# franioli/icepy4d

Hardware: AMD Instinct MI355X
Metric: matched stereo image-pairs/sec (4096 kpts, 1080p) (higher is better)
Workload: dtype f32

## Files before the change

icepy4d_amd/_lib.py:

```python
from __future__ import annotations

import ctypes as C
import os
import subprocess
from typing import Optional

_HERE = os.path.dirname(os.path.abspath(__file__))
CSRC = os.path.join(_HERE, "csrc")
LIB_PATH = os.environ.get("ICEMATCH_LIB") or os.path.join(CSRC, "libicematch.so")

_lib: Optional[C.CDLL] = None


class IcematchError(RuntimeError):

    def __init__(self, what: str, rc: int, message: str):
        super().__init__(f"{what} failed ({rc}): {message}")
        self.what, self.rc = what, rc


class LightGlueConf(C.Structure):
    _fields_ = [("depth_confidence", C.c_double), ("width_confidence", C.c_double),
                ("filter_threshold", C.c_double), ("n_layers", C.c_int), ("pruning_min_kpts", C.c_int)]

# ... 6 lines not shown
_I = C.c_int
_F = C.c_float
_D = C.c_double
_L = C.c_longlong

SIGNATURES = {
    "im_version": [],
    "im_ctx_create": [_I, C.POINTER(_P)],
    "im_ctx_destroy": [_P],
    "im_last_error": [_P],
    "im_ctx_reserve": [_P, _I, _I, _I, _I],
    "im_profile_begin": [_P],
    "im_profile_end": [_P, C.c_char_p, C.c_size_t],
    "im_set_tensor": [_P, C.c_char_p, C.c_char_p, _P, C.c_size_t],
    "im_finalize_weights": [_P, C.c_char_p],
    "im_superpoint_forward": [_P, _P, _I, _I, _I, _I, _I, _F, _I, _I, _I, _P, _P, _P, _P, _P],
    "im_superpoint_candidates": [_P, _I, _P, _P],
    "im_lightglue_forward": [_P, _P, _P, _P, _P, C.POINTER(LightGlueConf), _P, _P, _P, _P, _P],
    "im_lightglue_forward_pairs": [_P, _I, _P, _P, _P, _P, C.POINTER(LightGlueConf), _P, _P, _P, _P, _P],
    "im_pack_records": [_P, _I, _P, _P, _P, _P, _I, _P, _P, _P],
    "im_superglue_forward": [_P, _P, _P, _P, _P, _P, C.POINTER(SuperGlueConf), _P, _P, _P, _P],
    "im_pack_record": [_P, _P, _P, _P, _P, _I, _P, _P],
    "im_debug_read": [_P, C.c_char_p, _P, C.c_size_t, _P],
    "im_debug_clock_probe": [_P, _I, _P, _P],
    "im_debug_guard_failures": [],
    "im_debug_guard_selftest": [_P, _P],
    "im_debug_guards_check": [_P, _P],
    "im_pyr_down": [_P, _P, _P, _I, _I, _I, _I, _P],
    "im_pyr_up": [_P, _P, _P, _I, _I, _I, _I, _P],
    "im_gemm_nt": [_P, _P, _P, _P, _P, _I, _I, _I, _F, _I, _P],
    "im_ffn_fused": [_P, _I, _P, _P, _P, _P, _P, _P, _P, _P, _I, _I, _P, _P],
    "im_conv3x3": [_P, _P, _P, _P, _P, _I, _I, _I, _I, _I, _I, _I, _P],
    "im_conv3x3_winograd": [_P, _P, _P, _P, _P, _I, _I, _I, _I, _I, _I, _I, _P],
    "im_flash_attn": [_P, _P, _P, _P, _P, _P, _I, _I, _I, _I, _F, _P],
    "im_nms": [_P, _P, _P, _I, _I, _I, _I, _P],
    "im_select_topk": [_P, _P, _I, _I, _I, _I, _F, _I, _P, _P, _P, _P],
    "im_sample_descriptors": [_P, _P, _I, _I, _I, _P, _P, _P, _P],
    "im_assign_from_sim": [_P, _P, _I, _I, _I, _P, _P, _F, _P, _P, _P, _P, _P],
    "im_log_optimal_transport": [_P, _P, _I, _I, _I, _F, _I, _P, _P],
    "im_merge_tile_matches": [_P, _I, _I, _P, _P, _P, _P, _P, _P, _P, _P, _P, _P, _P, _P],
    "im_gather_rows": [_P, _P, _I, _P, _I, _P, _P],
    "im_ransac_fundamental": [_P, _P, _P, _I, _I, C.c_double, C.c_uint, _P, _P, _P, _P],
    "im_ransac_essential": [_P, _P, _P, _I, _I, C.c_double, C.c_uint, _P, _P, _P, _P],
    "im_triangulate_linear": [_P, _P, _P, _P, _P, _I, _P, _P],
    "im_forient": [_P, _P, _I, _I, _I, _I, _P, _P],
    "im_template_match_oc": [_P, _P, _I, _I, _P, _I, _I, _I, _P, _P, _I, _I, _I, _I, _P, _P],
# ... 85 lines not shown
```

icepy4d_amd/csrc/block.h:

```cpp
#pragma once
#include "ctx.h"

namespace im {

struct BlockFfn {
    int act = 0;
    const float* w0 = nullptr; const float* w0p = nullptr;
    const float* b0 = nullptr;
    const float* ln_g = nullptr; const float* ln_b = nullptr;
    const float* w3 = nullptr; const float* w3p = nullptr;
    const float* b3 = nullptr;
    const char* name_fused = nullptr; const char* name_ffn0 = nullptr; const char* name_ffn3 = nullptr;
};

int launch_block_proj(im_ctx* ctx, hipStream_t s, const char* name, const GemmArgs& g, const float* wp_layers, int layer);

int launch_block_tail(im_ctx* ctx, hipStream_t s, const AttnArgs& at, const BlockFfn& f, const GemmArgs& base, float* x);

}
```

icepy4d_amd/csrc/block.hip:

```cpp
#include "block.h"

#include "lg_misc.h"
#include "workspace.h"

namespace im {

int launch_block_proj(im_ctx* ctx, hipStream_t s, const char* name, const GemmArgs& g, const float* wp_layers, int layer) {
    if (env_is_1("IM_PROJ_TILED")) {
        IM_LAUNCH(ctx, name, s, launch_gemm(g, s));
        return 0;
    }
    GemmArgs r = g;
    r.wp = reinterpret_cast<const unsigned char*>(wp_layers) + (size_t)layer * g.N * 256 * 6;
    IM_LAUNCH(ctx, name, s, launch_proj_rows(r, s));
    return 0;
}

int launch_block_tail(im_ctx* ctx, hipStream_t s, const AttnArgs& at, const BlockFfn& f, const GemmArgs& base, float* x) {
    Workspace* ws = ctx->ws;
    const long xb = (long)base.m_max * 256, hb = (long)base.m_max * 512;
    IM_LAUNCH(ctx, "attn_kv_planes", s, launch_attn_planes(at, s));
    IM_LAUNCH(ctx, at.cross ? "flash_attn_cross" : "flash_attn_self", s, launch_flash_attn(at, s));
    static const bool unfused = env_is_1("IM_FFN_UNFUSED");
    if (!unfused) {
        FfnArgs a;
        a.act = f.act; a.x = x; a.x_bstride = xb; a.att = at.out; a.att_bstride = xb;
        a.w0p = f.w0p; a.b0 = f.b0; a.ln_g = f.ln_g; a.ln_b = f.ln_b; a.w3p = f.w3p; a.b3 = f.b3;
        a.m_max = base.m_max; a.batch = base.batch; a.m_ptr = base.m_ptr; a.active = base.active; a.pstride = base.pstride;
        IM_LAUNCH(ctx, f.name_fused, s, launch_ffn_fused(a, s));
        return 0;
    }
    {
        GemmArgs g = base;
        g.A = x; g.a_bstride = xb; g.lda = 256; g.A1 = at.out; g.a1_bstride = xb; g.lda1 = 256; g.ksplit = 256;
        g.W = f.w0; g.ldw = 512; g.bias = f.b0; g.N = 512; g.K = 512;
        g.C = ws->h; g.c_bstride = hb; g.ldc = 512; g.epi = f.act == 1 ? EPI_BIAS_RELU : EPI_BIAS;
        IM_LAUNCH(ctx, f.name_ffn0, s, launch_gemm(g, s));
    }
    if (f.act == 0)
        IM_LAUNCH(ctx, "lg_layernorm_gelu", s, launch_layernorm_gelu(ws->h, hb, ws->st, base.batch, base.m_max, f.ln_g, f.ln_b, s));
    {
        GemmArgs g = base;
        g.A = ws->h; g.a_bstride = hb; g.lda = 512; g.W = f.w3; g.ldw = 512; g.bias = f.b3; g.N = 256; g.K = 512;
        g.C = x; g.c_bstride = xb; g.ldc = 256; g.R = x; g.r_bstride = xb; g.ldr = 256; g.epi = EPI_BIAS_RESID;
// ... 7 lines not shown
```

icepy4d_amd/csrc/capi.hip:

```cpp
#include "ctx.h"
#include "lg_misc.h"
#include "sp_post.h"
#include "workspace.h"

#include <algorithm>
#include <cstdio>
#include <cstdlib>
#include <cstring>

using namespace im;

template <int N, typename F>
static hipError_t with_uploads(const float* const (&src)[N], const size_t (&sizes)[N], hipStream_t st, F&& launch) {
    float* d[N] = {};
    hipError_t e = hipSuccess;
    for (int i = 0; i < N && e == hipSuccess; ++i) {
        e = hipMalloc(&d[i], sizes[i] * sizeof(float));
        if (e == hipSuccess) e = hipMemcpy(d[i], src[i], sizes[i] * sizeof(float), hipMemcpyHostToDevice);
    }
    if (e == hipSuccess) e = launch(d);
    const hipError_t e2 = hipStreamSynchronize(st);
    for (int i = 0; i < N; ++i) hipFree(d[i]);
    return e != hipSuccess ? e : e2;
}
// ... 150 lines not shown
        first = false;
    }
    out += "}";
    if (!buf || out.size() + 1 > cap) return ctx->fail(-60, "im_profile_end: buffer too small (%zu needed)", out.size() + 1);
    memcpy(buf, out.c_str(), out.size() + 1);
    return 0;
}

int im_debug_read(im_ctx* ctx, const char* name, float* d_dst, size_t nfloats, void* stream) {
    IM_CHECK_CTX(ctx);
    Workspace* ws = ctx->ws;
    if (!ws || !name) return ctx->fail(-51, "im_debug_read: no workspace");
    const size_t K = (size_t)ctx->max_kpts;
    const std::string nm = name;
    const float* src = nullptr;
    size_t avail = 0;
    if (nm == "lg_x") { src = ws->x[ctx->dbg_cur]; avail = 2 * K * 256; }
    else if (nm == "lg_cos") { src = ws->cs[ctx->dbg_cur]; avail = 2 * K * 32; }
    else if (nm == "lg_sin") { src = ws->sn[ctx->dbg_cur]; avail = 2 * K * 32; }
    else if (nm == "sim") { src = ws->sim; avail = K * K; }
    else if (nm == "md") { src = ws->md; avail = 2 * K * 256; }
    else if (nm == "sp_smap") { src = ws->smap; avail = ws->smap_floats; }
    else if (nm == "sp_nms") { src = ws->nms; avail = ws->smap_floats; }
    else return ctx->fail(-61, "im_debug_read: unknown buffer '%s'", name);
    if (nfloats > avail) return ctx->fail(-62, "im_debug_read: %zu floats requested, %zu available", nfloats, avail);
    IM_HIP(ctx, hipMemcpyAsync(d_dst, src, nfloats * sizeof(float), hipMemcpyDeviceToDevice, (hipStream_t)stream));
    IM_HIP(ctx, hipStreamSynchronize((hipStream_t)stream));
    return 0;
}

int im_debug_clock_probe(im_ctx* ctx, int arm, double* h_out, void* stream) {
    IM_CHECK_CTX(ctx);
    hipStream_t s = (hipStream_t)stream;
    const size_t bytes = (size_t)CLOCK_PROBE_SLOTS * 2 * sizeof(unsigned long long);
    if (arm == 1) {
        IM_GROW(ctx, ctx->grow(ctx->scratch.clock[0], bytes, "clock_probe_attention"), -22, "im_debug_clock_probe: allocation failed");
        IM_GROW(ctx, ctx->grow(ctx->scratch.clock[1], bytes, "clock_probe_convolution"), -22, "im_debug_clock_probe: allocation failed");
        IM_HIP(ctx, hipMemsetAsync(ctx->scratch.clock[0].p, 0, bytes, s));
        IM_HIP(ctx, hipMemsetAsync(ctx->scratch.clock[1].p, 0, bytes, s));
        IM_HIP(ctx, hipStreamSynchronize(s));
        ctx->clock_armed = true;
        return 0;
    }
    if (!ctx->scratch.clock[0].p || !h_out) return ctx->fail(-51, "im_debug_clock_probe: not armed");
    std::vector<unsigned long long> h((size_t)CLOCK_PROBE_SLOTS * 2);
    const void* src[2] = {ctx->scratch.clock[0].p, ctx->scratch.clock[1].p};
    for (int c = 0; c < 2; ++c) {
        IM_HIP(ctx, hipMemcpyAsync(h.data(), src[c], bytes, hipMemcpyDeviceToHost, s));
        IM_HIP(ctx, hipStreamSynchronize(s));
// ... 145 lines not shown
```

icepy4d_amd/csrc/gemm.hip:

```cpp
#include "bf16x3.h"
#include "common.h"
#include "kernels.h"

namespace im {

template <int BM, int BN, int BK, int EPI, bool BX>
__global__ __launch_bounds__(256) void gemm_nt_kernel(GemmArgs a) {
    constexpr int LDS_LD = BK + 4;
    constexpr int WM = BM / 2, WN = BN / 2;
    constexpr int MB = WM / 32, NB = WN / 32;
    constexpr int F4 = BK / 4;
    constexpr int A_IT = BM * F4 / 256, B_IT = BN * F4 / 256;
    constexpr int XS = BK * 2 + 16, XPA = BM * XS, XPB = BN * XS;
    __shared__ __attribute__((aligned(16))) float smem[BX ? 3 * (XPA + XPB) / 4 : (BM + BN) * LDS_LD];
    float* sA = smem;
    float* sB = smem + BM * LDS_LD;
    unsigned char* const xA = reinterpret_cast<unsigned char*>(smem);
    unsigned char* const xB = xA + 3 * XPA;

    const int gm = (a.m_max + BM - 1) / BM;
    const int z = blockIdx.y;
    const int pair = a.pair_batched ? z : (z >> 1);
    if (a.active && a.active[pair * a.pstride] == 0) return;
    const int M = a.m_ptr ? a.m_ptr[a.pair_batched ? z * a.pstride : (z >> 1) * a.pstride + (z & 1)] : a.m_max;
// ... 185 lines not shown
                if (rope) {
                    const __amdgpu_buffer_rsrc_t rCs = make_rsrc(a.cs + (long)z * a.enc_bstride, (unsigned)M * 128u);
                    const __amdgpu_buffer_rsrc_t rSn = make_rsrc(a.sn + (long)z * a.enc_bstride, (unsigned)M * 128u);
                    const unsigned ve = (rowl * 32 + (d >> 1)) * 4u;
#pragma unroll
                    for (int r = 0; r < 16; ++r) {
                        const unsigned so = ((r & 3) + 8 * (r >> 2)) * 128u;
                        const float cs = __uint_as_float(__builtin_amdgcn_raw_buffer_load_b32(rCs, ve, so, 0));
                        const float sn = __uint_as_float(__builtin_amdgcn_raw_buffer_load_b32(rSn, ve, so, 0));
                        const float val = acc[i][j][r] + bv;
                        const float partner = __shfl_xor(val, 1);
                        const float outv = (d & 1) ? (val * cs) + (partner * sn) : (val * cs) + ((-partner) * sn);
                        __builtin_amdgcn_raw_buffer_store_b32(__float_as_uint(outv), rD, vo, ((r & 3) + 8 * (r >> 2)) * 256u, 0);
                    }
                } else {
#pragma unroll
                    for (int r = 0; r < 16; ++r)
                        __builtin_amdgcn_raw_buffer_store_b32(__float_as_uint(scale * (acc[i][j][r] + bv)), rD, vo, ((r & 3) + 8 * (r >> 2)) * 256u, 0);
                }
            }
        }
}

namespace pr {
constexpr int BM = 32, NT = 512;
constexpr int PS = 528;
constexpr int PLANE = BM * PS;
constexpr int LDS_BYTES = 3 * PLANE;
constexpr unsigned TILE_BYTES = (256 / 16) * 3 * 1024;
}

#ifdef IM_PSTAMP
__device__ unsigned long long g_pstamp[4096 * 16];
#define P_STAMP(i) { if (wave == 0) { const unsigned long long ts_ = __builtin_amdgcn_s_memtime(); const int b_ = blockIdx.y * gridDim.x + blockIdx.x; if (lane == 0 && b_ < 4096) g_pstamp[b_ * 16 + (i)] = ts_; } }
extern "C" int im_debug_pstamps(unsigned long long* host, size_t n) {
    return (int)hipMemcpyFromSymbol(host, HIP_SYMBOL(g_pstamp), n * sizeof(unsigned long long));
}
#else
#define P_STAMP(i)
#endif

template <int EPI, int TILES>
__global__ __launch_bounds__(pr::NT, 4) void proj_rows_kernel(GemmArgs a) {
    using namespace pr;
    static_assert(EPI == EPI_QKV_ROPE || EPI == EPI_HEADS_QV, "the two projections of a LightGlue block");
    extern __shared__ __attribute__((aligned(16))) unsigned char psm[];
    const int z = blockIdx.y, pair = z >> 1;
    if (a.active && a.active[pair * a.pstride] == 0) return;
    const int M = a.m_ptr ? a.m_ptr[pair * a.pstride + (z & 1)] : a.m_max;
    const int m0 = blockIdx.x * BM;
    if (m0 >= M) return;
    const int tid = threadIdx.x, lane = tid & 63;
    const int wave = __builtin_amdgcn_readfirstlane(tid >> 6);
    const int c = lane & 31, hh = lane >> 5;
    const __amdgpu_buffer_rsrc_t rX = make_rsrc(a.A + (long)z * a.a_bstride, (unsigned)M * 1024u);
    const __amdgpu_buffer_rsrc_t rW = make_rsrc(a.wp, (unsigned)a.N * 256u * 6u);

    P_STAMP(0)
    u32x4 b0[3], b1[3], b2[3], b3[3];
#define PR_LOAD(b_, s_)                                                                                                          \
    {                                                                                                                            \
        const bool in_ = (s_) < TILES * 16;                                                                                      \
        const unsigned so_ = in_ ? (unsigned)((((s_) >> 4) * 8 + wave)) * TILE_BYTES + (unsigned)(((s_) & 15) * 3) * 1024u : 0u;   \
        const unsigned vo_ = in_ ? lane * 16u : 0x80000000u;     \
        _Pragma("unroll") for (int g = 0; g < 3; ++g) b_[g] = __builtin_amdgcn_raw_buffer_load_b128(rW, vo_, so_ + (unsigned)g * 1024u, 0); \
    }
    PR_LOAD(b0, 0)
    PR_LOAD(b1, 1)
    PR_LOAD(b2, 2)
    {
        float4 v[4];
#pragma unroll
        for (int i = 0; i < 4; ++i) {
            const int idx = tid + i * NT;
            v[i] = buf_load4(rX, (unsigned)((m0 + (idx >> 6)) * 256 + (idx & 63) * 4) * 4u, 0);
        }
#pragma unroll
        for (int i = 0; i < 4; ++i) {
            const int idx = tid + i * NT;
            unsigned h0, m0_, l0, h1, m1, l1;
            split2(v[i].x, v[i].y, h0, m0_, l0);
            split2(v[i].z, v[i].w, h1, m1, l1);
            unsigned char* d = psm + (idx >> 6) * PS + (idx & 63) * 8;
            *reinterpret_cast<u32x2*>(d) = u32x2{h0, h1};
            *reinterpret_cast<u32x2*>(d + PLANE) = u32x2{m0_, m1};
            *reinterpret_cast<u32x2*>(d + 2 * PLANE) = u32x2{l0, l1};
        }
    }
    __syncthreads();
    P_STAMP(1)

#define PR_SIX(b_, kc_)                                                                                              \
    {                                                                                                                \
        const unsigned char* ap = psm + c * PS + ((kc_) * 16 + hh * 8) * 2;                                          \
        const u32x4 ah = *reinterpret_cast<const u32x4*>(ap), am = *reinterpret_cast<const u32x4*>(ap + PLANE),   \
                     al = *reinterpret_cast<const u32x4*>(ap + 2 * PLANE);                                          \
        acc = mfma_bf(ah, b_[2], acc);                                                                              \
        acc = mfma_bf(al, b_[0], acc);                                                                              \
        acc = mfma_bf(am, b_[1], acc);                                                                              \
        acc = mfma_bf(ah, b_[1], acc);                                                                              \
        acc = mfma_bf(am, b_[0], acc);                                                                              \
        acc = mfma_bf(ah, b_[0], acc);                                                                              \
    }
#pragma unroll 1
    for (int j = 0; j < TILES; ++j) {
        const int tile = j * 8 + wave;
        f32x16 acc;
#pragma unroll
        for (int r = 0; r < 16; ++r) acc[r] = 0.f;
#pragma unroll 1
        for (int kc = 0; kc < 16; kc += 4) {
            const int s_ = j * 16 + kc;
            PR_LOAD(b3, s_ + 3)
            __builtin_amdgcn_sched_barrier(0);
            PR_SIX(b0, kc)
            __builtin_amdgcn_sched_barrier(0);
            PR_LOAD(b0, s_ + 4)
            __builtin_amdgcn_sched_barrier(0);
            PR_SIX(b1, kc + 1)
            __builtin_amdgcn_sched_barrier(0);
            PR_LOAD(b1, s_ + 5)
            __builtin_amdgcn_sched_barrier(0);
            PR_SIX(b2, kc + 2)
            __builtin_amdgcn_sched_barrier(0);
            PR_LOAD(b2, s_ + 6)
            __builtin_amdgcn_sched_barrier(0);
            PR_SIX(b3, kc + 3)
            __builtin_amdgcn_sched_barrier(0);
        }
        P_STAMP(2 + 2 * j)
        const int colbase = tile * 32;
        const int col = colbase + c;
        const float bv = a.bias ? a.bias[col] : 0.f;
        const unsigned rowl = m0 + 4 * hh;
        const int which = colbase >> 8, hd = colbase & 255;
        float* dst = a.q;
        if constexpr (EPI == EPI_QKV_ROPE) dst = which == 0 ? a.q : (which == 1 ? a.k : a.v);
        if constexpr (EPI == EPI_HEADS_QV) dst = which ? a.v : a.q;
        const __amdgpu_buffer_rsrc_t rD = make_rsrc(dst + (long)z * a.head_bstride + (long)(hd >> 6) * a.head_stride, (unsigned)M * 256u);
        const int d = (hd & 63) + c;
        const unsigned vo = (rowl * 64 + d) * 4u;
        float scale = a.alpha;
        if constexpr (EPI == EPI_QKV_ROPE) scale = 1.f;
        if constexpr (EPI == EPI_HEADS_QV) scale = which ? 1.f : a.alpha;
        const bool rope = EPI == EPI_QKV_ROPE && which < 2 && a.cs;
        if (rope) {
            const __amdgpu_buffer_rsrc_t rCs = make_rsrc(a.cs + (long)z * a.enc_bstride, (unsigned)M * 128u);
            const __amdgpu_buffer_rsrc_t rSn = make_rsrc(a.sn + (long)z * a.enc_bstride, (unsigned)M * 128u);
            const unsigned ve = (rowl * 32 + (d >> 1)) * 4u;
#pragma unroll
            for (int r = 0; r < 16; ++r) {
                const unsigned so = ((r & 3) + 8 * (r >> 2)) * 128u;
                const float cs = __uint_as_float(__builtin_amdgcn_raw_buffer_load_b32(rCs, ve, so, 0));
                const float sn = __uint_as_float(__builtin_amdgcn_raw_buffer_load_b32(rSn, ve, so, 0));
                const float val = acc[r] + bv;
                const float partner = __shfl_xor(val, 1);
                const float outv = (d & 1) ? (val * cs) + (partner * sn) : (val * cs) + ((-partner) * sn);
                __builtin_amdgcn_raw_buffer_store_b32(__float_as_uint(outv), rD, vo, ((r & 3) + 8 * (r >> 2)) * 256u, 0);
            }
        } else {
#pragma unroll
            for (int r = 0; r < 16; ++r)
                __builtin_amdgcn_raw_buffer_store_b32(__float_as_uint(scale * (acc[r] + bv)), rD, vo, ((r & 3) + 8 * (r >> 2)) * 256u, 0);
        }
        P_STAMP(3 + 2 * j)
    }
#undef PR_LOAD
#undef PR_SIX
}

template <int EPI, int TILES>
static hipError_t launch_proj_rows_t(const GemmArgs& a, hipStream_t s) {
    const dim3 grid((a.m_max + pr::BM - 1) / pr::BM, a.batch), block(pr::NT);
    return launch_dyn_lds<proj_rows_kernel<EPI, TILES>>(grid, block, pr::LDS_BYTES, s, a);
}

hipError_t launch_proj_rows(const GemmArgs& a, hipStream_t s) {
    if (!a.wp || a.K != 256 || a.lda != 256 || a.A1 || a.sel || a.w_bstride || a.n_ptr || a.pair_batched) return hipErrorInvalidValue;
    if (a.m_max <= 0 || a.batch <= 0) return hipSuccess;
    if (a.epi == EPI_QKV_ROPE && a.N == 768) return launch_proj_rows_t<EPI_QKV_ROPE, 3>(a, s);
    if (a.epi == EPI_HEADS_QV && a.N == 512) return launch_proj_rows_t<EPI_HEADS_QV, 2>(a, s);
    return hipErrorInvalidValue;
}

hipError_t launch_gemm(const GemmArgs& a, hipStream_t s) {
    if (a.K % 32 != 0 || (a.A1 && a.ksplit % 64 != 0)) return hipErrorInvalidValue;
    const int bm = a.big_tile ? 128 : 64, bn = bm;
    dim3 grid(((a.N + bn - 1) / bn) * ((a.m_max + bm - 1) / bm), a.batch), block(256);
    if (grid.x == 0) return hipSuccess;
#define IM_GEMM_CASE(E)                                                                  \
    case E:                                                                              \
// ... 23 lines not shown
```

icepy4d_amd/csrc/kernels.h:

```cpp
#pragma once
#include <hip/hip_runtime.h>
#include <stdint.h>
#include <cstdlib>
#include <vector>

#include "common.h"

namespace im {

inline bool env_is_1(const char* name) {
    const char* e = getenv(name);
    return e && e[0] == '1';
}
inline int env_int(const char* name) {
    const char* e = getenv(name);
    return e ? atoi(e) : 0;
}

inline hipError_t current_device(int* dev) {
    if (hipError_t e = hipGetDevice(dev); e != hipSuccess) return e;
    return (*dev < 0 || *dev >= IM_MAX_DEVICES) ? hipErrorInvalidDevice : hipSuccess;
}
inline hipError_t device_cu_count(int* n) {
    static int n_cu[IM_MAX_DEVICES] = {0};
// ... 34 lines not shown

struct GemmArgs {
    const float* A = nullptr;  long a_bstride = 0;  int lda = 0;
    const float* A1 = nullptr; long a1_bstride = 0; int lda1 = 0; int ksplit = 0;
    const float* W = nullptr;  int ldw = 0; long w_bstride = 0;
    const float* bias = nullptr;
    const int* sel = nullptr; long w_sel_stride = 0; long bias_sel_stride = 0;
    int N = 0, K = 0;
    int m_max = 0;
    const int* m_ptr = nullptr;
    const int* n_ptr = nullptr;
    const int* active = nullptr;
    int pstride = 2;
    int pair_batched = 0;
    int batch = 1;
    float alpha = 1.f;
    float* C = nullptr; long c_bstride = 0; int ldc = 0;
    const float* R = nullptr; long r_bstride = 0; int ldr = 0;
    float* q = nullptr; float* k = nullptr; float* v = nullptr; long head_bstride = 0; long head_stride = 0;
    const float* cs = nullptr; const float* sn = nullptr; long enc_bstride = 0;
    int epi = EPI_BIAS;
    int big_tile = 0;
    int bx = 0;
    const void* wp = nullptr;
};
hipError_t launch_gemm(const GemmArgs& a, hipStream_t s);
hipError_t launch_proj_rows(const GemmArgs& a, hipStream_t s);

struct FfnArgs {
    int act = 0;
    float* x = nullptr; long x_bstride = 0;
    const float* att = nullptr; long att_bstride = 0;
    const float* w0p = nullptr; const float* b0 = nullptr;
    const float* ln_g = nullptr; const float* ln_b = nullptr;
    const float* w3p = nullptr; const float* b3 = nullptr;
    int m_max = 0; int batch = 1;
    const int* m_ptr = nullptr;
    const int* active = nullptr;
    int pstride = 2;
};
hipError_t launch_ffn_fused(const FfnArgs& a, hipStream_t s);
std::vector<float> pack_frag_weights(const float* w, int n, int k);

struct AttnArgs {
    const float* q = nullptr; const float* k = nullptr; const float* v = nullptr;
    long bstride = 0; long hstride = 0;
    float* out = nullptr; long out_bstride = 0; int ldo = 256;
    const int* n_ptr = nullptr;
    int pstride = 2;
    int n_max = 0; int batch = 2; int heads = 4; int cross = 0;
    float scale = 1.f;
    const int* active = nullptr;
    float* part = nullptr;
    int* counters = nullptr;
    void* planes = nullptr;
    int f32_form = 0;
    unsigned long long* clock = nullptr;
};
static constexpr int CLOCK_PROBE_SLOTS = 4096;
static constexpr int ATTN_MAX_SPLIT = 4;
inline size_t attn_part_floats(int n_max, int batch, int heads) { return (size_t)ATTN_MAX_SPLIT * batch * heads * n_max * 66; }
inline size_t attn_planes_bytes(int n_max, int batch, int heads) { return (size_t)2 * batch * heads * n_max * 384; }
inline size_t attn_counter_ints(int n_max, int batch, int heads) { return (size_t)batch * heads * ((n_max + 127) / 128); }
bool attn_f32_form(const AttnArgs& a);
hipError_t launch_flash_attn(const AttnArgs& a, hipStream_t s);
hipError_t launch_attn_planes(const AttnArgs& a, hipStream_t s);
hipError_t launch_flash_attn_bx(const AttnArgs& a, hipStream_t s);

struct ConvArgs {
    const float* in = nullptr;
    const float* w = nullptr;
    const float* bias = nullptr;
    float* out = nullptr;
    int B = 1, H = 0, W = 0, Cin = 0, Cout = 0;
    int pool = 0;
    int relu = 1;
    const uint8_t* img = nullptr;
    int img_channels = 1;
// ... 16 lines not shown
```

icepy4d_amd/csrc/lightglue.hip:

```cpp
#include "block.h"
#include "lg_misc.h"
#include "workspace.h"

using namespace im;

static constexpr int ST_INTS = (int)(sizeof(LGState) / sizeof(int));

static int lg_block(im_ctx* ctx, hipStream_t s, int NI, int layer, bool cross, float* x, const float* cs, const float* sn) {
    Workspace* ws = ctx->ws;
    const LightGlueW& W = ctx->lg;
    const int K = ctx->max_kpts;
    const long xb = (long)K * 256;
    const int* n_ptr = ws->st->n;
    const int* active = &ws->st->active;
    GemmArgs base;
    base.m_max = K; base.m_ptr = n_ptr; base.active = active; base.pstride = ST_INTS; base.batch = NI; base.bx = 1;
    AttnArgs at;
    at.q = ws->q; at.k = cross ? ws->q : ws->k; at.v = ws->v; at.hstride = (long)K * 64; at.bstride = (long)K * 256;
    at.out = ws->att; at.out_bstride = xb; at.ldo = 256; at.n_ptr = n_ptr; at.pstride = ST_INTS; at.n_max = K; at.batch = NI; at.heads = 4;
    at.cross = cross ? 1 : 0; at.active = active; at.part = ws->attn_part; at.counters = ws->attn_cnt; at.planes = ws->attn_planes; at.clock = ctx->clock_of(0);
    GemmArgs g = base;
    g.A = x; g.a_bstride = xb; g.lda = 256; g.ldw = 256; g.K = 256;
    g.q = ws->q; g.v = ws->v; g.head_bstride = (long)K * 256; g.head_stride = (long)K * 64; g.big_tile = NI >= 4;
    if (!cross) {
        g.W = W.qkv_w + (long)layer * 768 * 256; g.bias = W.qkv_b + (long)layer * 768; g.N = 768; g.epi = EPI_QKV_ROPE;
        g.k = ws->k; g.cs = cs; g.sn = sn; g.enc_bstride = (long)K * 32;
        if (int rc = launch_block_proj(ctx, s, "lg_qkv_rope_gemm", g, W.qkv_wp, layer)) return rc;
        at.scale = 0.125f;
    } else {
        g.W = W.cqv_w + (long)layer * 512 * 256; g.bias = W.cqv_b + (long)layer * 512; g.N = 512; g.epi = EPI_HEADS_QV;
        g.alpha = (float)0.35355339059327373;
        if (int rc = launch_block_proj(ctx, s, "lg_proj_gemm", g, W.cqv_wp, layer)) return rc;
        at.scale = 1.f;
    }
    const LightGlueW::Ffn& F = cross ? W.cross_ffn : W.self_ffn;
    BlockFfn f;
    f.w0 = F.w0 + (long)layer * 512 * 512; f.w0p = F.w0p + (long)layer * 512 * 512 * 3 / 2; f.b0 = F.b0 + (long)layer * 512;
    f.ln_g = F.ln_g + (long)layer * 512; f.ln_b = F.ln_b + (long)layer * 512;
    f.w3 = F.w3 + (long)layer * 256 * 512; f.w3p = F.w3p + (long)layer * 256 * 512 * 3 / 2; f.b3 = F.b3 + (long)layer * 256;
    f.name_fused = "lg_ffn_fused"; f.name_ffn0 = "lg_ffn0_gemm"; f.name_ffn3 = "lg_ffn3_gemm";
    return launch_block_tail(ctx, s, at, f, base, x);
}

static int lightglue_forward(im_ctx* ctx, int n_pairs, const float* d_kpts, const float* d_desc, const int32_t* d_n, const float* h_size,
                             const im_lightglue_conf* conf, int32_t* d_matches, float* d_mscores, int32_t* d_prune, int32_t* d_info,
                             void* stream) {
    IM_CHECK_CTX(ctx);
    if (!ctx->lg.ready) return ctx->fail(-50, "im_lightglue_forward: weights not finalized");
    Workspace* ws = ctx->ws;
    if (!ws) return ctx->fail(-51, "im_lightglue_forward: call im_ctx_reserve first");
    if (n_pairs < 1 || n_pairs > ws->n_pairs || n_pairs > 64)
        return ctx->fail(-53, "im_lightglue_forward: %d pairs, the workspace was reserved for %d (max_images / 2)", n_pairs, ws->n_pairs);
    hipStream_t s = (hipStream_t)stream;
    const LightGlueW& W = ctx->lg;
    const int K = ctx->max_kpts;
// ... 98 lines not shown
```

include/icematch.h:

```cpp
#ifndef ICEMATCH_H
#define ICEMATCH_H

#include <stddef.h>
#include <stdint.h>

#ifdef __cplusplus
extern "C" {
#endif

typedef struct im_ctx im_ctx;

int im_version(void);
int im_ctx_create(int device, im_ctx** out);
void im_ctx_destroy(im_ctx* ctx);
const char* im_last_error(im_ctx* ctx);
int im_ctx_reserve(im_ctx* ctx, int max_h, int max_w, int max_images, int max_kpts);

int im_profile_begin(im_ctx* ctx);
int im_profile_end(im_ctx* ctx, char* buf, size_t cap);

int im_set_tensor(im_ctx* ctx, const char* model, const char* key, const float* h_data, size_t numel);
int im_finalize_weights(im_ctx* ctx, const char* model);

int im_superpoint_forward(im_ctx* ctx, const uint8_t* d_img, int n_images, int h, int w, int channels,
// ... 10 lines not shown
} im_lightglue_conf;
int im_lightglue_forward(im_ctx* ctx, const float* d_kpts, const float* d_desc, const int32_t* d_n,
                         const float* h_size, const im_lightglue_conf* conf,
                         int32_t* d_matches, float* d_mscores, int32_t* d_prune, int32_t* d_info, void* stream);

int im_lightglue_forward_pairs(im_ctx* ctx, int n_pairs, const float* d_kpts, const float* d_desc, const int32_t* d_n,
                               const float* h_size, const im_lightglue_conf* conf, int32_t* d_matches, float* d_mscores,
                               int32_t* d_prune, int32_t* d_info, void* stream);

typedef struct {
    int sinkhorn_iterations;
    double match_threshold;
    int n_layers;
} im_superglue_conf;
int im_superglue_forward(im_ctx* ctx, const float* d_kpts, const float* d_scores, const float* d_desc,
                         const int32_t* d_n, const float* h_shape, const im_superglue_conf* conf,
                         int32_t* d_matches, float* d_mscores, int32_t* d_info, void* stream);

int im_pack_record(im_ctx* ctx, const int32_t* d_n, const int32_t* d_matches0, const float* d_mscores0,
                   const int32_t* d_info, int epoch, int32_t* d_record, void* stream);
int im_pack_records(im_ctx* ctx, int n_pairs, const int32_t* d_n, const int32_t* d_matches, const float* d_mscores,
                    const int32_t* d_info, int first_epoch, int32_t* d_records, const float* d_kpts, void* stream);
int im_debug_read(im_ctx* ctx, const char* name, float* d_dst, size_t nfloats, void* stream);
int im_debug_clock_probe(im_ctx* ctx, int arm, double* h_out, void* stream);
int im_debug_guard_failures(void);
int im_debug_guard_selftest(im_ctx* ctx, void* stream);
int im_debug_guards_check(im_ctx* ctx, void* stream);

int im_gemm_nt(im_ctx* ctx, const float* d_a, const float* d_w, const float* d_bias, float* d_c,
               int m, int n, int k, float alpha, int big_tile, void* stream);
int im_ffn_fused(im_ctx* ctx, int act, float* d_x, const float* d_att, const float* h_w0, const float* h_b0, const float* h_ln_g,
                   const float* h_ln_b, const float* h_w3, const float* h_b3, int n_images, int n_rows, const int32_t* d_n, void* stream);
int im_conv3x3(im_ctx* ctx, const float* d_in, const float* h_weight, const float* h_bias, float* d_out,
               int b, int h, int w, int cin, int cout, int relu, int pool, void* stream);
int im_conv3x3_winograd(im_ctx* ctx, const float* d_in, const float* h_weight, const float* h_bias, float* d_out,
                        int b, int h, int w, int cin, int cout, int relu, int pool, void* stream);
int im_flash_attn(im_ctx* ctx, const float* d_q, const float* d_k, const float* d_v, float* d_out,
                  const int32_t* d_n, int n_max, int batch, int heads, int cross, float scale, void* stream);
int im_nms(im_ctx* ctx, const float* d_scores, float* d_out, int n_images, int h, int w, int radius, void* stream);
int im_select_topk(im_ctx* ctx, const float* d_nms, int n_images, int h, int w, int border, float threshold,
                   int max_kpts, float* d_kpts, float* d_scores, int32_t* d_n, void* stream);
int im_sample_descriptors(im_ctx* ctx, const float* d_dense_raw, int n_images, int hc, int wc,
                          const float* d_kpts, const int32_t* d_n, float* d_desc, void* stream);
int im_assign_from_sim(im_ctx* ctx, const float* d_sim, int m, int n, int ld, const float* d_z0, const float* d_z1,
                       float threshold, int32_t* d_m0, int32_t* d_m1, float* d_ms0, float* d_ms1, void* stream);
int im_log_optimal_transport(im_ctx* ctx, const float* d_scores, int m, int n, int ld, float bin_score, int iters,
// ... 64 lines not shown
```

Before: 164.8.

## Fuse K/V bf16x3 plane packing into LightGlue projection epilogue

The projection GEMM epilogue now writes K and V straight into the split bf16x3 plane layout that flash attention reads, so the separate attn_kv_planes kernel is skipped when the projection has already filled the planes. This removes one kernel launch and a full re-read and re-write of K/V per layer. The f32 K/V stores are dropped on that path, and the projection body is moved into a shared header templated on the epilogue. A debug fill hook and an env switch are added for validation, which leaves correctness dependent on the plane layout matching exactly what the attention kernel expects.

Result: no change. 165.3 (median of 4 runs) (+0.3%).

```diff
diff --git a/icepy4d_amd/_lib.py b/icepy4d_amd/_lib.py
--- a/icepy4d_amd/_lib.py
+++ b/icepy4d_amd/_lib.py
@@ -52,6 +52,7 @@
     "im_superglue_forward": [_P, _P, _P, _P, _P, _P, C.POINTER(SuperGlueConf), _P, _P, _P, _P],
     "im_pack_record": [_P, _P, _P, _P, _P, _I, _P, _P],
     "im_debug_read": [_P, C.c_char_p, _P, C.c_size_t, _P],
+    "im_debug_fill": [_P, C.c_char_p, _I, _P],
     "im_debug_clock_probe": [_P, _I, _P, _P],
     "im_debug_guard_failures": [],
     "im_debug_guard_selftest": [_P, _P],
diff --git a/icepy4d_amd/csrc/block.h b/icepy4d_amd/csrc/block.h
--- a/icepy4d_amd/csrc/block.h
+++ b/icepy4d_amd/csrc/block.h
@@ -13,7 +13,7 @@
     const char* name_fused = nullptr; const char* name_ffn0 = nullptr; const char* name_ffn3 = nullptr;
 };
 
-int launch_block_proj(im_ctx* ctx, hipStream_t s, const char* name, const GemmArgs& g, const float* wp_layers, int layer);
+int launch_block_proj(im_ctx* ctx, hipStream_t s, const char* name, const GemmArgs& g, const float* wp_layers, int layer, AttnArgs* at = nullptr);
 
 int launch_block_tail(im_ctx* ctx, hipStream_t s, const AttnArgs& at, const BlockFfn& f, const GemmArgs& base, float* x);
 
diff --git a/icepy4d_amd/csrc/block.hip b/icepy4d_amd/csrc/block.hip
--- a/icepy4d_amd/csrc/block.hip
+++ b/icepy4d_amd/csrc/block.hip
@@ -5,13 +5,20 @@
 
 namespace im {
 
-int launch_block_proj(im_ctx* ctx, hipStream_t s, const char* name, const GemmArgs& g, const float* wp_layers, int layer) {
+int launch_block_proj(im_ctx* ctx, hipStream_t s, const char* name, const GemmArgs& g, const float* wp_layers, int layer, AttnArgs* at) {
     if (env_is_1("IM_PROJ_TILED")) {
         IM_LAUNCH(ctx, name, s, launch_gemm(g, s));
         return 0;
     }
     GemmArgs r = g;
     r.wp = reinterpret_cast<const unsigned char*>(wp_layers) + (size_t)layer * g.N * 256 * 6;
+    const char* sw = getenv("IM_PROJ_PLANES");
+    if (at && at->planes && !attn_f32_form(*at) && at->heads == 4 && at->n_max == g.m_max && at->batch == g.batch && !(sw && sw[0] == '0')) {
+        r.planes = at->planes;
+        IM_LAUNCH(ctx, name, s, launch_proj_rows_planes(r, s));
+        at->planes_filled = 1;
+        return 0;
+    }
     IM_LAUNCH(ctx, name, s, launch_proj_rows(r, s));
     return 0;
 }
@@ -19,7 +26,7 @@
 int launch_block_tail(im_ctx* ctx, hipStream_t s, const AttnArgs& at, const BlockFfn& f, const GemmArgs& base, float* x) {
     Workspace* ws = ctx->ws;
     const long xb = (long)base.m_max * 256, hb = (long)base.m_max * 512;
-    IM_LAUNCH(ctx, "attn_kv_planes", s, launch_attn_planes(at, s));
+    if (!at.planes_filled) IM_LAUNCH(ctx, "attn_kv_planes", s, launch_attn_planes(at, s));
     IM_LAUNCH(ctx, at.cross ? "flash_attn_cross" : "flash_attn_self", s, launch_flash_attn(at, s));
     static const bool unfused = env_is_1("IM_FFN_UNFUSED");
     if (!unfused) {
diff --git a/icepy4d_amd/csrc/capi.hip b/icepy4d_amd/csrc/capi.hip
--- a/icepy4d_amd/csrc/capi.hip
+++ b/icepy4d_amd/csrc/capi.hip
@@ -196,9 +196,20 @@
     else if (nm == "md") { src = ws->md; avail = 2 * K * 256; }
     else if (nm == "sp_smap") { src = ws->smap; avail = ws->smap_floats; }
     else if (nm == "sp_nms") { src = ws->nms; avail = ws->smap_floats; }
+    else if (nm == "attn_planes") { src = reinterpret_cast<const float*>(ws->attn_planes); avail = attn_planes_bytes((int)K, 2 * ws->n_pairs, 4) / 4; }
     else return ctx->fail(-61, "im_debug_read: unknown buffer '%s'", name);
     if (nfloats > avail) return ctx->fail(-62, "im_debug_read: %zu floats requested, %zu available", nfloats, avail);
     IM_HIP(ctx, hipMemcpyAsync(d_dst, src, nfloats * sizeof(float), hipMemcpyDeviceToDevice, (hipStream_t)stream));
+    IM_HIP(ctx, hipStreamSynchronize((hipStream_t)stream));
+    return 0;
+}
+
+int im_debug_fill(im_ctx* ctx, const char* name, int byte_value, void* stream) {
+    IM_CHECK_CTX(ctx);
+    Workspace* ws = ctx->ws;
+    if (!ws || !name) return ctx->fail(-51, "im_debug_fill: no workspace");
+    if (std::string(name) != "attn_planes") return ctx->fail(-61, "im_debug_fill: unknown buffer '%s'", name);
+    IM_HIP(ctx, hipMemsetAsync(ws->attn_planes, byte_value, attn_planes_bytes(ctx->max_kpts, 2 * ws->n_pairs, 4), (hipStream_t)stream));
     IM_HIP(ctx, hipStreamSynchronize((hipStream_t)stream));
     return 0;
 }
diff --git a/icepy4d_amd/csrc/gemm.hip b/icepy4d_amd/csrc/gemm.hip
--- a/icepy4d_amd/csrc/gemm.hip
+++ b/icepy4d_amd/csrc/gemm.hip
@@ -231,14 +231,6 @@
         }
 }
 
-namespace pr {
-constexpr int BM = 32, NT = 512;
-constexpr int PS = 528;
-constexpr int PLANE = BM * PS;
-constexpr int LDS_BYTES = 3 * PLANE;
-constexpr unsigned TILE_BYTES = (256 / 16) * 3 * 1024;
-}
-
 #ifdef IM_PSTAMP
 __device__ unsigned long long g_pstamp[4096 * 16];
 #define P_STAMP(i) { if (wave == 0) { const unsigned long long ts_ = __builtin_amdgcn_s_memtime(); const int b_ = blockIdx.y * gridDim.x + blockIdx.x; if (lane == 0 && b_ < 4096) g_pstamp[b_ * 16 + (i)] = ts_; } }
@@ -249,133 +241,13 @@
 #define P_STAMP(i)
 #endif
 
+}
+#include "proj_rows.h"
+namespace im {
+
 template <int EPI, int TILES>
 __global__ __launch_bounds__(pr::NT, 4) void proj_rows_kernel(GemmArgs a) {
-    using namespace pr;
-    static_assert(EPI == EPI_QKV_ROPE || EPI == EPI_HEADS_QV, "the two projections of a LightGlue block");
-    extern __shared__ __attribute__((aligned(16))) unsigned char psm[];
-    const int z = blockIdx.y, pair = z >> 1;
-    if (a.active && a.active[pair * a.pstride] == 0) return;
-    const int M = a.m_ptr ? a.m_ptr[pair * a.pstride + (z & 1)] : a.m_max;
-    const int m0 = blockIdx.x * BM;
-    if (m0 >= M) return;
-    const int tid = threadIdx.x, lane = tid & 63;
-    const int wave = __builtin_amdgcn_readfirstlane(tid >> 6);
-    const int c = lane & 31, hh = lane >> 5;
-    const __amdgpu_buffer_rsrc_t rX = make_rsrc(a.A + (long)z * a.a_bstride, (unsigned)M * 1024u);
-    const __amdgpu_buffer_rsrc_t rW = make_rsrc(a.wp, (unsigned)a.N * 256u * 6u);
-
-    P_STAMP(0)
-    u32x4 b0[3], b1[3], b2[3], b3[3];
-#define PR_LOAD(b_, s_)                                                                                                          \
-    {                                                                                                                            \
-        const bool in_ = (s_) < TILES * 16;                                                                                      \
-        const unsigned so_ = in_ ? (unsigned)((((s_) >> 4) * 8 + wave)) * TILE_BYTES + (unsigned)(((s_) & 15) * 3) * 1024u : 0u;   \
-        const unsigned vo_ = in_ ? lane * 16u : 0x80000000u;     \
-        _Pragma("unroll") for (int g = 0; g < 3; ++g) b_[g] = __builtin_amdgcn_raw_buffer_load_b128(rW, vo_, so_ + (unsigned)g * 1024u, 0); \
-    }
-    PR_LOAD(b0, 0)
-    PR_LOAD(b1, 1)
-    PR_LOAD(b2, 2)
-    {
-        float4 v[4];
-#pragma unroll
-        for (int i = 0; i < 4; ++i) {
-            const int idx = tid + i * NT;
-            v[i] = buf_load4(rX, (unsigned)((m0 + (idx >> 6)) * 256 + (idx & 63) * 4) * 4u, 0);
-        }
-#pragma unroll
-        for (int i = 0; i < 4; ++i) {
-            const int idx = tid + i * NT;
-            unsigned h0, m0_, l0, h1, m1, l1;
-            split2(v[i].x, v[i].y, h0, m0_, l0);
-            split2(v[i].z, v[i].w, h1, m1, l1);
-            unsigned char* d = psm + (idx >> 6) * PS + (idx & 63) * 8;
-            *reinterpret_cast<u32x2*>(d) = u32x2{h0, h1};
-            *reinterpret_cast<u32x2*>(d + PLANE) = u32x2{m0_, m1};
-            *reinterpret_cast<u32x2*>(d + 2 * PLANE) = u32x2{l0, l1};
-        }
-    }
-    __syncthreads();
-    P_STAMP(1)
-
-#define PR_SIX(b_, kc_)                                                                                              \
-    {                                                                                                                \
-        const unsigned char* ap = psm + c * PS + ((kc_) * 16 + hh * 8) * 2;                                          \
-        const u32x4 ah = *reinterpret_cast<const u32x4*>(ap), am = *reinterpret_cast<const u32x4*>(ap + PLANE),   \
-                     al = *reinterpret_cast<const u32x4*>(ap + 2 * PLANE);                                          \
-        acc = mfma_bf(ah, b_[2], acc);                                                                              \
-        acc = mfma_bf(al, b_[0], acc);                                                                              \
-        acc = mfma_bf(am, b_[1], acc);                                                                              \
-        acc = mfma_bf(ah, b_[1], acc);                                                                              \
-        acc = mfma_bf(am, b_[0], acc);                                                                              \
-        acc = mfma_bf(ah, b_[0], acc);                                                                              \
-    }
-#pragma unroll 1
-    for (int j = 0; j < TILES; ++j) {
-        const int tile = j * 8 + wave;
-        f32x16 acc;
-#pragma unroll
-        for (int r = 0; r < 16; ++r) acc[r] = 0.f;
-#pragma unroll 1
-        for (int kc = 0; kc < 16; kc += 4) {
-            const int s_ = j * 16 + kc;
-            PR_LOAD(b3, s_ + 3)
-            __builtin_amdgcn_sched_barrier(0);
-            PR_SIX(b0, kc)
-            __builtin_amdgcn_sched_barrier(0);
-            PR_LOAD(b0, s_ + 4)
-            __builtin_amdgcn_sched_barrier(0);
-            PR_SIX(b1, kc + 1)
-            __builtin_amdgcn_sched_barrier(0);
-            PR_LOAD(b1, s_ + 5)
-            __builtin_amdgcn_sched_barrier(0);
-            PR_SIX(b2, kc + 2)
-            __builtin_amdgcn_sched_barrier(0);
-            PR_LOAD(b2, s_ + 6)
-            __builtin_amdgcn_sched_barrier(0);
-            PR_SIX(b3, kc + 3)
-            __builtin_amdgcn_sched_barrier(0);
-        }
-        P_STAMP(2 + 2 * j)
-        const int colbase = tile * 32;
-        const int col = colbase + c;
-        const float bv = a.bias ? a.bias[col] : 0.f;
-        const unsigned rowl = m0 + 4 * hh;
-        const int which = colbase >> 8, hd = colbase & 255;
-        float* dst = a.q;
-        if constexpr (EPI == EPI_QKV_ROPE) dst = which == 0 ? a.q : (which == 1 ? a.k : a.v);
-        if constexpr (EPI == EPI_HEADS_QV) dst = which ? a.v : a.q;
-        const __amdgpu_buffer_rsrc_t rD = make_rsrc(dst + (long)z * a.head_bstride + (long)(hd >> 6) * a.head_stride, (unsigned)M * 256u);
-        const int d = (hd & 63) + c;
-        const unsigned vo = (rowl * 64 + d) * 4u;
-        float scale = a.alpha;
-        if constexpr (EPI == EPI_QKV_ROPE) scale = 1.f;
-        if constexpr (EPI == EPI_HEADS_QV) scale = which ? 1.f : a.alpha;
-        const bool rope = EPI == EPI_QKV_ROPE && which < 2 && a.cs;
-        if (rope) {
-            const __amdgpu_buffer_rsrc_t rCs = make_rsrc(a.cs + (long)z * a.enc_bstride, (unsigned)M * 128u);
-            const __amdgpu_buffer_rsrc_t rSn = make_rsrc(a.sn + (long)z * a.enc_bstride, (unsigned)M * 128u);
-            const unsigned ve = (rowl * 32 + (d >> 1)) * 4u;
-#pragma unroll
-            for (int r = 0; r < 16; ++r) {
-                const unsigned so = ((r & 3) + 8 * (r >> 2)) * 128u;
-                const float cs = __uint_as_float(__builtin_amdgcn_raw_buffer_load_b32(rCs, ve, so, 0));
-                const float sn = __uint_as_float(__builtin_amdgcn_raw_buffer_load_b32(rSn, ve, so, 0));
-                const float val = acc[r] + bv;
-                const float partner = __shfl_xor(val, 1);
-                const float outv = (d & 1) ? (val * cs) + (partner * sn) : (val * cs) + ((-partner) * sn);
-                __builtin_amdgcn_raw_buffer_store_b32(__float_as_uint(outv), rD, vo, ((r & 3) + 8 * (r >> 2)) * 256u, 0);
-            }
-        } else {
-#pragma unroll
-            for (int r = 0; r < 16; ++r)
-                __builtin_amdgcn_raw_buffer_store_b32(__float_as_uint(scale * (acc[r] + bv)), rD, vo, ((r & 3) + 8 * (r >> 2)) * 256u, 0);
-        }
-        P_STAMP(3 + 2 * j)
-    }
-#undef PR_LOAD
-#undef PR_SIX
+    proj_rows_body<EPI, TILES, ProjEpiF32>(a);
 }
 
 template <int EPI, int TILES>
diff --git a/icepy4d_amd/csrc/kernels.h b/icepy4d_amd/csrc/kernels.h
--- a/icepy4d_amd/csrc/kernels.h
+++ b/icepy4d_amd/csrc/kernels.h
@@ -80,10 +80,12 @@
     int epi = EPI_BIAS;
     int big_tile = 0;
     int bx = 0;
+    void* planes = nullptr;
     const void* wp = nullptr;
 };
 hipError_t launch_gemm(const GemmArgs& a, hipStream_t s);
 hipError_t launch_proj_rows(const GemmArgs& a, hipStream_t s);
+hipError_t launch_proj_rows_planes(const GemmArgs& a, hipStream_t s);
 
 struct FfnArgs {
     int act = 0;
@@ -112,6 +114,7 @@
     float* part = nullptr;
     int* counters = nullptr;
     void* planes = nullptr;
+    int planes_filled = 0;
     int f32_form = 0;
     unsigned long long* clock = nullptr;
 };
diff --git a/icepy4d_amd/csrc/lightglue.hip b/icepy4d_amd/csrc/lightglue.hip
--- a/icepy4d_amd/csrc/lightglue.hip
+++ b/icepy4d_amd/csrc/lightglue.hip
@@ -25,12 +25,12 @@
     if (!cross) {
         g.W = W.qkv_w + (long)layer * 768 * 256; g.bias = W.qkv_b + (long)layer * 768; g.N = 768; g.epi = EPI_QKV_ROPE;
         g.k = ws->k; g.cs = cs; g.sn = sn; g.enc_bstride = (long)K * 32;
-        if (int rc = launch_block_proj(ctx, s, "lg_qkv_rope_gemm", g, W.qkv_wp, layer)) return rc;
+        if (int rc = launch_block_proj(ctx, s, "lg_qkv_rope_gemm", g, W.qkv_wp, layer, &at)) return rc;
         at.scale = 0.125f;
     } else {
         g.W = W.cqv_w + (long)layer * 512 * 256; g.bias = W.cqv_b + (long)layer * 512; g.N = 512; g.epi = EPI_HEADS_QV;
         g.alpha = (float)0.35355339059327373;
-        if (int rc = launch_block_proj(ctx, s, "lg_proj_gemm", g, W.cqv_wp, layer)) return rc;
+        if (int rc = launch_block_proj(ctx, s, "lg_proj_gemm", g, W.cqv_wp, layer, &at)) return rc;
         at.scale = 1.f;
     }
     const LightGlueW::Ffn& F = cross ? W.cross_ffn : W.self_ffn;
diff --git a/icepy4d_amd/csrc/proj_planes.hip b/icepy4d_amd/csrc/proj_planes.hip
--- /dev/null
+++ b/icepy4d_amd/csrc/proj_planes.hip
@@ -0,0 +1,24 @@
+#include "proj_rows.h"
+
+namespace im {
+
+template <int EPI, int TILES>
+__global__ __launch_bounds__(pr::NT, 4) void proj_rows_planes_kernel(GemmArgs a) {
+    proj_rows_body<EPI, TILES, ProjEpiPlanes>(a);
+}
+
+template <int EPI, int TILES>
+static hipError_t launch_proj_rows_planes_t(const GemmArgs& a, hipStream_t s) {
+    const dim3 grid((a.m_max + pr::BM - 1) / pr::BM, a.batch), block(pr::NT);
+    return launch_dyn_lds<proj_rows_planes_kernel<EPI, TILES>>(grid, block, pr::LDS_BYTES, s, a);
+}
+
+hipError_t launch_proj_rows_planes(const GemmArgs& a, hipStream_t s) {
+    if (!a.planes || !a.wp || a.K != 256 || a.lda != 256 || a.A1 || a.sel || a.w_bstride || a.n_ptr || a.pair_batched) return hipErrorInvalidValue;
+    if (a.m_max <= 0 || a.batch <= 0) return hipSuccess;
+    if (a.epi == EPI_QKV_ROPE && a.N == 768) return launch_proj_rows_planes_t<EPI_QKV_ROPE, 3>(a, s);
+    if (a.epi == EPI_HEADS_QV && a.N == 512) return launch_proj_rows_planes_t<EPI_HEADS_QV, 2>(a, s);
+    return hipErrorInvalidValue;
+}
+
+}
diff --git a/icepy4d_amd/csrc/proj_rows.h b/icepy4d_amd/csrc/proj_rows.h
--- /dev/null
+++ b/icepy4d_amd/csrc/proj_rows.h
@@ -0,0 +1,208 @@
+#pragma once
+#include "bf16x3.h"
+#include "common.h"
+#include "kernels.h"
+
+#ifndef P_STAMP
+#define P_STAMP(i)
+#endif
+
+namespace im {
+
+namespace pr {
+constexpr int BM = 32, NT = 512;
+constexpr int PS = 528;
+constexpr int PLANE = BM * PS;
+constexpr int LDS_BYTES = 3 * PLANE;
+constexpr unsigned TILE_BYTES = (256 / 16) * 3 * 1024;
+}
+
+template <int EPI, class Put>
+__device__ __forceinline__ void proj_tile_values(const GemmArgs& a, const f32x16& acc, int tile, int z, int M, int m0, int c, int hh, Put put) {
+    const int colbase = tile * 32;
+    const int col = colbase + c;
+    const float bv = a.bias ? a.bias[col] : 0.f;
+    const unsigned rowl = m0 + 4 * hh;
+    const int which = colbase >> 8, hd = colbase & 255;
+    const int d = (hd & 63) + c;
+    float scale = a.alpha;
+    if constexpr (EPI == EPI_QKV_ROPE) scale = 1.f;
+    if constexpr (EPI == EPI_HEADS_QV) scale = which ? 1.f : a.alpha;
+    const bool rope = EPI == EPI_QKV_ROPE && which < 2 && a.cs;
+    if (rope) {
+        const __amdgpu_buffer_rsrc_t rCs = make_rsrc(a.cs + (long)z * a.enc_bstride, (unsigned)M * 128u);
+        const __amdgpu_buffer_rsrc_t rSn = make_rsrc(a.sn + (long)z * a.enc_bstride, (unsigned)M * 128u);
+        const unsigned ve = (rowl * 32 + (d >> 1)) * 4u;
+#pragma unroll
+        for (int r = 0; r < 16; ++r) {
+            const unsigned so = ((r & 3) + 8 * (r >> 2)) * 128u;
+            const float cs = __uint_as_float(__builtin_amdgcn_raw_buffer_load_b32(rCs, ve, so, 0));
+            const float sn = __uint_as_float(__builtin_amdgcn_raw_buffer_load_b32(rSn, ve, so, 0));
+            const float val = acc[r] + bv;
+            const float partner = __shfl_xor(val, 1);
+            const float outv = (d & 1) ? (val * cs) + (partner * sn) : (val * cs) + ((-partner) * sn);
+            put(r, outv);
+        }
+    } else {
+#pragma unroll
+        for (int r = 0; r < 16; ++r) put(r, scale * (acc[r] + bv));
+    }
+}
+
+template <int EPI>
+struct ProjDstF32 {
+    __amdgpu_buffer_rsrc_t rD;
+    unsigned vo;
+    __device__ __forceinline__ ProjDstF32(const GemmArgs& a, int tile, int z, int M, int m0, int c, int hh) {
+        const int colbase = tile * 32;
+        const int which = colbase >> 8, hd = colbase & 255;
+        float* dst = a.q;
+        if constexpr (EPI == EPI_QKV_ROPE) dst = which == 0 ? a.q : (which == 1 ? a.k : a.v);
+        if constexpr (EPI == EPI_HEADS_QV) dst = which ? a.v : a.q;
+        rD = make_rsrc(dst + (long)z * a.head_bstride + (long)(hd >> 6) * a.head_stride, (unsigned)M * 256u);
+        vo = ((m0 + 4 * hh) * 64 + (hd & 63) + c) * 4u;
+    }
+    __device__ __forceinline__ void store(int r, float v) const {
+        __builtin_amdgcn_raw_buffer_store_b32(__float_as_uint(v), rD, vo, ((r & 3) + 8 * (r >> 2)) * 256u, 0);
+    }
+};
+
+struct ProjEpiF32 {
+    template <int EPI>
+    static __device__ __forceinline__ void tile(const GemmArgs& a, const f32x16& acc, int tile, int z, int M, int m0, int c, int hh) {
+        const ProjDstF32<EPI> D(a, tile, z, M, m0, c, hh);
+        proj_tile_values<EPI>(a, acc, tile, z, M, m0, c, hh, [&](int r, float v) { D.store(r, v); });
+    }
+};
+
+struct ProjEpiPlanes {
+    static __device__ __forceinline__ float lane_xor1(float x) {
+        return __int_as_float(__builtin_amdgcn_update_dpp(0, __float_as_int(x), 0xB1, 0xF, 0xF, true));
+    }
+    template <int EPI>
+    static __device__ __forceinline__ void tile(const GemmArgs& a, const f32x16& acc, int tile, int z, int M, int m0, int c, int hh) {
+        const int colbase = tile * 32;
+        const int which = colbase >> 8, hd = colbase & 255;
+        float out[16];
+        if (which == 0) {
+            const ProjDstF32<EPI> D(a, tile, z, M, m0, c, hh);
+            proj_tile_values<EPI>(a, acc, tile, z, M, m0, c, hh, [&](int r, float v) { out[r] = v; D.store(r, v); });
+            if constexpr (EPI == EPI_QKV_ROPE) return;
+        } else {
+            proj_tile_values<EPI>(a, acc, tile, z, M, m0, c, hh, [&](int r, float v) { out[r] = v; });
+        }
+        const int kv = EPI == EPI_QKV_ROPE ? which - 1 : which;
+        const __amdgpu_buffer_rsrc_t rP = make_rsrc(static_cast<unsigned char*>(a.planes) + (((long)kv * a.batch + z) * 4 + (hd >> 6)) * a.m_max * 384, (unsigned)M * 384u);
+        const bool odd = c & 1;
+        const unsigned vo = (m0 + 4 * hh + (odd ? 16 : 0)) * 384u + (unsigned)(((hd & 63) + c) >> 1) * 4u;
+#pragma unroll
+        for (int r = 0; r < 8; ++r) {
+            const float mine = odd ? out[r + 8] : out[r];
+            const float got = lane_xor1(odd ? out[r] : out[r + 8]);
+            unsigned h, m, l;
+            split2(odd ? got : mine, odd ? mine : got, h, m, l);
+            const unsigned so = ((r & 3) + 8 * (r >> 2)) * 384u;
+            __builtin_amdgcn_raw_buffer_store_b32(h, rP, vo + so, 0, 0);
+            __builtin_amdgcn_raw_buffer_store_b32(m, rP, vo + so + 128u, 0, 0);
+            __builtin_amdgcn_raw_buffer_store_b32(l, rP, vo + so + 256u, 0, 0);
+        }
+    }
+};
+
+template <int EPI, int TILES, class Epi>
+__device__ __forceinline__ void proj_rows_body(const GemmArgs& a) {
+    using namespace pr;
+    static_assert(EPI == EPI_QKV_ROPE || EPI == EPI_HEADS_QV, "the two projections of a LightGlue block");
+    extern __shared__ __attribute__((aligned(16))) unsigned char psm[];
+    const int z = blockIdx.y, pair = z >> 1;
+    if (a.active && a.active[pair * a.pstride] == 0) return;
+    const int M = a.m_ptr ? a.m_ptr[pair * a.pstride + (z & 1)] : a.m_max;
+    const int m0 = blockIdx.x * BM;
+    if (m0 >= M) return;
+    const int tid = threadIdx.x, lane = tid & 63;
+    const int wave = __builtin_amdgcn_readfirstlane(tid >> 6);
+    const int c = lane & 31, hh = lane >> 5;
+    const __amdgpu_buffer_rsrc_t rX = make_rsrc(a.A + (long)z * a.a_bstride, (unsigned)M * 1024u);
+    const __amdgpu_buffer_rsrc_t rW = make_rsrc(a.wp, (unsigned)a.N * 256u * 6u);
+
+    P_STAMP(0)
+    u32x4 b0[3], b1[3], b2[3], b3[3];
+#define PR_LOAD(b_, s_)                                                                                                          \
+    {                                                                                                                            \
+        const bool in_ = (s_) < TILES * 16;                                                                                      \
+        const unsigned so_ = in_ ? (unsigned)((((s_) >> 4) * 8 + wave)) * TILE_BYTES + (unsigned)(((s_) & 15) * 3) * 1024u : 0u;   \
+        const unsigned vo_ = in_ ? lane * 16u : 0x80000000u;     \
+        _Pragma("unroll") for (int g = 0; g < 3; ++g) b_[g] = __builtin_amdgcn_raw_buffer_load_b128(rW, vo_, so_ + (unsigned)g * 1024u, 0); \
+    }
+    PR_LOAD(b0, 0)
+    PR_LOAD(b1, 1)
+    PR_LOAD(b2, 2)
+    {
+        float4 v[4];
+#pragma unroll
+        for (int i = 0; i < 4; ++i) {
+            const int idx = tid + i * NT;
+            v[i] = buf_load4(rX, (unsigned)((m0 + (idx >> 6)) * 256 + (idx & 63) * 4) * 4u, 0);
+        }
+#pragma unroll
+        for (int i = 0; i < 4; ++i) {
+            const int idx = tid + i * NT;
+            unsigned h0, m0_, l0, h1, m1, l1;
+            split2(v[i].x, v[i].y, h0, m0_, l0);
+            split2(v[i].z, v[i].w, h1, m1, l1);
+            unsigned char* d = psm + (idx >> 6) * PS + (idx & 63) * 8;
+            *reinterpret_cast<u32x2*>(d) = u32x2{h0, h1};
+            *reinterpret_cast<u32x2*>(d + PLANE) = u32x2{m0_, m1};
+            *reinterpret_cast<u32x2*>(d + 2 * PLANE) = u32x2{l0, l1};
+        }
+    }
+    __syncthreads();
+    P_STAMP(1)
+
+#define PR_SIX(b_, kc_)                                                                                              \
+    {                                                                                                                \
+        const unsigned char* ap = psm + c * PS + ((kc_) * 16 + hh * 8) * 2;                                          \
+        const u32x4 ah = *reinterpret_cast<const u32x4*>(ap), am = *reinterpret_cast<const u32x4*>(ap + PLANE),   \
+                     al = *reinterpret_cast<const u32x4*>(ap + 2 * PLANE);                                          \
+        acc = mfma_bf(ah, b_[2], acc);                                                                              \
+        acc = mfma_bf(al, b_[0], acc);                                                                              \
+        acc = mfma_bf(am, b_[1], acc);                                                                              \
+        acc = mfma_bf(ah, b_[1], acc);                                                                              \
+        acc = mfma_bf(am, b_[0], acc);                                                                              \
+        acc = mfma_bf(ah, b_[0], acc);                                                                              \
+    }
+#pragma unroll 1
+    for (int j = 0; j < TILES; ++j) {
+        const int tile = j * 8 + wave;
+        f32x16 acc;
+#pragma unroll
+        for (int r = 0; r < 16; ++r) acc[r] = 0.f;
+#pragma unroll 1
+        for (int kc = 0; kc < 16; kc += 4) {
+            const int s_ = j * 16 + kc;
+            PR_LOAD(b3, s_ + 3)
+            __builtin_amdgcn_sched_barrier(0);
+            PR_SIX(b0, kc)
+            __builtin_amdgcn_sched_barrier(0);
+            PR_LOAD(b0, s_ + 4)
+            __builtin_amdgcn_sched_barrier(0);
+            PR_SIX(b1, kc + 1)
+            __builtin_amdgcn_sched_barrier(0);
+            PR_LOAD(b1, s_ + 5)
+            __builtin_amdgcn_sched_barrier(0);
+            PR_SIX(b2, kc + 2)
+            __builtin_amdgcn_sched_barrier(0);
+            PR_LOAD(b2, s_ + 6)
+            __builtin_amdgcn_sched_barrier(0);
+            PR_SIX(b3, kc + 3)
+            __builtin_amdgcn_sched_barrier(0);
+        }
+        P_STAMP(2 + 2 * j)
+        Epi::template tile<EPI>(a, acc, tile, z, M, m0, c, hh);
+        P_STAMP(3 + 2 * j)
+    }
+#undef PR_LOAD
+#undef PR_SIX
+}
+
+}
diff --git a/include/icematch.h b/include/icematch.h
--- a/include/icematch.h
+++ b/include/icematch.h
@@ -56,6 +56,7 @@
 int im_pack_records(im_ctx* ctx, int n_pairs, const int32_t* d_n, const int32_t* d_matches, const float* d_mscores,
                     const int32_t* d_info, int first_epoch, int32_t* d_records, const float* d_kpts, void* stream);
 int im_debug_read(im_ctx* ctx, const char* name, float* d_dst, size_t nfloats, void* stream);
+int im_debug_fill(im_ctx* ctx, const char* name, int byte_value, void* stream);
 int im_debug_clock_probe(im_ctx* ctx, int arm, double* h_out, void* stream);
 int im_debug_guard_failures(void);
 int im_debug_guard_selftest(im_ctx* ctx, void* stream);
```
